# yonahd/krr

Measured on AMD Instinct MI355X. Metric: container-series/sec right-sized (7d@1m) + % of HBM BW, 1/2/4/8 MI355X, higher is better.
Workload: dtype f64; 1 GPU; config2: 10000 containers/rank x 5 pods x 10080 slots (7d@1m), NaN-gapped dense; percentile_mode=linear, cpu_percentile=99, memory_buffer=max x 1.05 (exact decimal, host), containers=10000, slots_per_rank=1008000000, parallelism=shard1 (contiguous container ranges, RCCL gather of 32-B records), records=page-locked host memory, written by the launch

## Files before the change

krr_amd/csrc/krr_geom.h:

```cpp
#pragma once

#include <stdint.h>

#include "krr_plan.h"

namespace krr {

#define KRR_GEOM KRR_HD inline __attribute__((always_inline))

constexpr int kChunkUnits = kUnroll * kWave;

struct SegGeom {
    int64_t a0, a1;
    int64_t s0;
    int64_t i0;
    int64_t nunits;
    int64_t nfull;
    int32_t rem;
    bool head, tail;
    bool part;
    KRR_GEOM bool partial() const { return part; }
    KRR_GEOM int64_t nch() const { return nfull + (partial() ? 1 : 0); }
    KRR_GEOM uint32_t padding() const {
        return partial() ? (uint32_t)(2 * kChunkUnits - 2 * rem - (head ? 1 : 0) - (tail ? 1 : 0)) : 0u;
    }
    KRR_GEOM int64_t slot(int64_t ci, int u, int l) const { return s0 + 2 * (ci * kChunkUnits + u * kWave + l); }
    KRR_GEOM bool edge(int64_t ci, int u, int l) const {
        return partial() && ci == nfull && u == kUnroll - 1 && l == kWave - 1;
    }
};

KRR_GEOM SegGeom seg_geom(int64_t beg, int64_t end) {
    int64_t a0 = (beg + 1) & ~(int64_t)1;
    if (a0 > end) a0 = end;
    int64_t a1 = end & ~(int64_t)1;
    if (a1 < a0) a1 = a0;
    const int64_t i0 = a0 >> 1;
    const int64_t nunits = (a1 >> 1) - i0;
    const int64_t nfull = nunits / kChunkUnits;
    const int64_t rem = nunits - nfull * kChunkUnits;
    const bool head = a0 > beg, tail = a1 < end;
    const bool part = rem > 0 || head || tail;
    return SegGeom{a0, a1, a0 - beg, i0, nunits, nfull, (int32_t)rem, head, tail, part};
}

struct SegCursor {
    uint32_t full;
    int64_t base;
    int lane;
    KRR_GEOM SegCursor(const SegGeom& g, int lane_) : full((uint32_t)g.nfull), base(g.s0), lane(lane_) {}
    KRR_GEOM bool partial() const { return full == 0; }
    KRR_GEOM bool edge_row(int u) const { return partial() && u == kUnroll - 1; }
    KRR_GEOM bool edge(int u) const { return edge_row(u) && lane == kWave - 1; }
    KRR_GEOM int64_t row_base(int u) const { return base + 2 * kWave * u; }
    KRR_GEOM void next() {
        base += 2 * kChunkUnits;
        --full;
    }
};

}
```

krr_amd/csrc/krr_kernels.hip:

```cpp
#include <hip/hip_runtime.h>

#include <stdint.h>
#include <stdio.h>
#include <string.h>

#include <dlfcn.h>
#include <sched.h>
#include <time.h>
#include <unistd.h>
#include <rccl/rccl.h>

#include <new>
#include <type_traits>

#include "krr_amd.h"
#include "krr_device.h"
#include "krr_plan.h"
#include "krr_geom.h"
#include "krr_json.h"

#ifndef KRR_STREAM_DEPTH
#define KRR_STREAM_DEPTH 2
#endif
#ifndef KRR_WSEL_LONG_DEPTH
// ... 1779 lines not shown
    W.fail = 0;
    W.set_window(kKeyNegInf, kKeyPosInf);
#ifdef KRR_DIAG
    for (int d = 0; d < D_WORDS; ++d) W.diag[d] = 0;
    KRR_DIAG_T0(t_begin);
#endif
    int64_t b = beg, e = end;
    asm volatile("" : "+s"(b), "+s"(e));
    const uint32_t pad =
        stream_segment<true, WindowProc<INLINE_FALLBACK>, INLINE_FALLBACK ? KRR_WSEL_LONG_DEPTH : KRR_ONE_SITE_DEPTH>(
            A.vals, b, e, W, lane);
    __syncthreads();
    const uint64_t nnan = W.nan_total() - pad;
    const uint64_t n = A.gaps ? (uint64_t)L - nnan : (uint64_t)L;
    uint32_t flags = 0;
    double result = bitsd(kQuietNaN);
    bool done = false;
#ifdef KRR_DIAG
    KRR_DIAG_T0(t_final);
#endif
    if (W.fail) {
    } else if (n == 0) {
        flags = KRR_FLAG_EMPTY;
        done = true;
    } else if (nnan && !A.gaps) {
        flags = KRR_FLAG_NAN;
        done = true;
    } else {
        const Ranks R = ranks_for(A, n);
        const uint64_t below = W.below_total();
        if (below <= (uint64_t)R.r0 && (uint64_t)R.r1 < below + W.cnt) {
            uint64_t k0, k1;
            if (W.point) {
                k0 = k1 = W.lo;
            } else {
                W.sp.cnt = W.cnt;
                W.sp.bad = 0;
                uint64_t mn = W.lo, mx = W.hi;
                if (W.shrinks == 0) W.sp.buf_minmax(mn, mx);
                const uint32_t Rt = (uint32_t)(W.cnt - ((uint64_t)R.r0 - below));
                if (R.r1 != R.r0) {
                    W.sp.kth_pair(Rt, -1, mn, mx, k0, k1);
                } else {
                    k0 = k1 = W.sp.kth_largest(Rt, mn, mx);
                }
            }
            if (!W.sp.bad) {
                result = finish_value(A, R, k0, k1, beg, end, lane);
                done = true;
            }
        }
    }
#ifdef KRR_DIAG
    {
        const unsigned long long t_end = __builtin_amdgcn_s_memtime();
        W.diag[D_TOTAL] = t_end - t_begin;
        W.diag[D_FINAL] = t_end - t_final;
        W.diag[D_NFALLBACK] = done ? 0ull : 1ull;
        W.diag[D_INSERTED] = W.cnt;
        if (lane == 0 && g_diag)
            for (int d = 0; d < D_WORDS; ++d) g_diag[(size_t)s * D_WORDS + d] = W.diag[d];
    }
#endif
    __syncthreads();
    if (!done) {
        if (lane == 0 && A.stats) atomicAdd(A.stats, 1ull);
        if constexpr (INLINE_FALLBACK) {
            hselect_segment(A, s, smem, lane);
        } else if (lane == 0) {
            A.fail_list[atomicAdd(A.fail_count, 1u)] = s;
        }
        return;
    }
    write_result(A, s, result, n, flags, lane);
    __syncthreads();
}

template <bool LONG>
__device__ __forceinline__ void mid_select_segment(const SelectArgs& A, int64_t s, unsigned char* smem, int lane) {
    if constexpr (KRR_WSEL) wselect_segment<LONG>(A, s, smem, lane);
    else hselect_segment(A, s, smem, lane);
}

__global__ __launch_bounds__(64, KRR_HSEL_WAVES_PER_SIMD) void k_hselect_list(SelectArgs A) {
    extern __shared__ __attribute__((aligned(16))) unsigned char smem[];
    const unsigned int n = __builtin_nontemporal_load(A.fail_count);
    for (unsigned int i = blockIdx.x; i < n; i += gridDim.x) hselect_segment(A, A.fail_list[i], smem, threadIdx.x);
}

enum { SEL_SINGLE = 0, SEL_WINDOW = 1, SEL_WINDOW_LONG = 2 };
constexpr int window_waves(bool longseg) {
    return !KRR_WSEL ? KRR_HSEL_WAVES_PER_SIMD : (longseg ? KRR_HSEL_WAVES_PER_SIMD : KRR_WSEL_WAVES_PER_SIMD);
}
template <int KIND>
__global__ __launch_bounds__(64, KIND == SEL_SINGLE ? KRR_SELECT_WAVES_PER_SIMD : window_waves(KIND == SEL_WINDOW_LONG))
void k_select(SelectArgs A) {
    extern __shared__ __attribute__((aligned(16))) unsigned char smem[];
    if (KIND != SEL_SINGLE && A.fail_reset && blockIdx.x == 0 && threadIdx.x == 0) *A.fail_reset = 0;
    for (int64_t s = blockIdx.x; s < A.S; s += gridDim.x) {
        if constexpr (KIND != SEL_SINGLE) mid_select_segment<KIND == SEL_WINDOW_LONG>(A, xcd_item(s, A.S, A.remap), smem, threadIdx.x);
        else select_segment(A, xcd_item(s, A.S, A.remap), smem, threadIdx.x);
    }
}

struct WindowExportArgs {
    SelectArgs A;
    double ext;
    uint32_t key_cap;
    krr_window_hdr* hdr;
    uint64_t* keys;
};

template <bool LONG>
__device__ __forceinline__ void window_export_segment(const WindowExportArgs& X, int64_t s, unsigned char* smem,
                                                      int lane) {
    const SelectArgs& A = X.A;
    const int64_t beg = A.offs[s], end = A.offs[s + 1];
    const int64_t L = end - beg;
    WindowProc<LONG, true> W;
    W.buf = reinterpret_cast<uint64_t*>(smem + kSelectLdsFixed);
    W.sp.buf = W.buf;
    W.sp.H = reinterpret_cast<uint32_t*>(smem);
    W.sp.small = reinterpret_cast<uint64_t*>(smem + 1024);
    W.sp.lane = lane;
    W.sp.flip = 0;
    W.sp.cnt = 0;
    W.sp.bad = 0;
    W.lane = lane;
    W.cap = A.wcap;
    W.shrinks = 0;
    W.cnt = 0;
    W.below_u = W.nan_u = 0;
    W.below_l = W.nan_l = W.negnan_l = 0;
    W.below_extra = 0;
    W.seen = 0;
    W.L = L;
    W.p_num = A.p_num;
    W.p_den = A.p_den;
    W.fail = 0;
    W.ext_u = X.ext;
    W.set_window(kKeyNegInf, kKeyPosInf);
    int64_t b = (int64_t)uni64((uint64_t)beg), e = (int64_t)uni64((uint64_t)end);
    asm volatile("" : "+s"(b), "+s"(e));
    const uint32_t pad = stream_segment<true, WindowProc<LONG, true>, LONG ? KRR_WSEL_LONG_DEPTH : KRR_ONE_SITE_DEPTH>(
        A.vals, b, e, W, lane);
    __syncthreads();
    const uint64_t nnan = W.fail ? 0 : W.nan_total() - pad;
    const uint64_t n = A.gaps ? (uint64_t)L - nnan : (uint64_t)L;
    const bool has_nan = nnan && !A.gaps;
    if (!W.fail && n > 0 && !has_nan) W.export_shrink(X.key_cap);
    uint32_t flags = 0;
    if (has_nan) W.cnt = 0;
    if (W.fail || (!W.point && W.cnt > X.key_cap)) flags |= KRR_WIN_FAIL;
    if (has_nan) flags |= KRR_FLAG_NAN;
    if (W.point) flags |= KRR_WIN_POINT;
    if (!(flags & (KRR_WIN_FAIL | KRR_WIN_POINT))) {
        uint64_t* row = X.keys + (size_t)s * X.key_cap;
        for (uint32_t i = lane; i < W.cnt; i += kWave) row[i] = W.buf[i];
    }
    const uint64_t below = W.below_total();
    if (lane == 0) {
        krr_window_hdr h;
        h.lo = W.lo;
        h.hi = W.hi;
        h.below = (int64_t)below;
        h.n = (int64_t)n;
        h.cnt = W.cnt;
        h.flags = flags;
        X.hdr[s] = h;
    }
    __syncthreads();
}

template <bool LONG>
__global__ __launch_bounds__(64, window_waves(LONG)) void k_window_export(WindowExportArgs X) {
    extern __shared__ __attribute__((aligned(16))) unsigned char smem[];
    for (int64_t s = blockIdx.x; s < X.A.S; s += gridDim.x) window_export_segment<LONG>(X, xcd_item(s, X.A.S, X.A.remap), smem, threadIdx.x);
}

struct OpAdd64 {
    __device__ uint64_t operator()(uint64_t a, uint64_t b) const { return a + b; }
};
__device__ __forceinline__ uint64_t wave_sum_u64(uint64_t x) {
    return lane_bcast64(wave_scan64(x, 0ull, OpAdd64{}), kWave - 1);
}

struct WindowMergeArgs {
    SelectArgs A;
    int32_t slices;
    int64_t stride;
    const krr_window_hdr* hdr;
    const uint64_t* keys;
    int64_t key_cap;
    unsigned int* miss_count;
};

__global__ __launch_bounds__(64) void k_window_merge(WindowMergeArgs M) {
    extern __shared__ __attribute__((aligned(16))) unsigned char smem[];
    const int lane = threadIdx.x;
    const SelectArgs& A = M.A;
    uint64_t* buf = reinterpret_cast<uint64_t*>(smem + kSelectLdsFixed);
    for (int64_t s = blockIdx.x; s < A.S; s += gridDim.x) {
        const bool has = lane < M.slices;
        krr_window_hdr h;
        if (has) {
            h = M.hdr[(int64_t)lane * M.stride + s];
        } else {
            h.lo = 0;
            h.hi = ~0ull;
            h.below = h.n = 0;
            h.cnt = h.flags = 0;
        }
        const uint64_t n = wave_sum_u64((uint64_t)h.n);
        const uint64_t Lk = wave_max_u64(h.lo), Hk = wave_min_u64(h.hi);
        const bool any_nan = ballot((h.flags & KRR_FLAG_NAN) != 0) != 0;
        const bool any_fail =
            ballot((h.flags & KRR_WIN_FAIL) != 0 || (!(h.flags & KRR_WIN_POINT) && h.cnt > M.key_cap)) != 0;
        uint32_t flags = 0;
        double result = bitsd(kQuietNaN);
        bool miss = false;
        if (any_nan) {
            flags = KRR_FLAG_NAN;
        } else if (n == 0) {
            flags = KRR_FLAG_EMPTY;
        } else if (!rule_covers((int64_t)n, A.ktab, A.ktab_len)) {
            flags = KRR_FLAG_CAPACITY;
        } else if (any_fail || Lk > Hk) {
            miss = true;
        } else {
            const Ranks R = ranks_for(A, n);
            uint64_t cb = wave_sum_u64((uint64_t)h.below);
            uint32_t inr = 0, inr_point = 0;
#pragma unroll 1
            for (int j = 0; j < M.slices; ++j) {
                const uint64_t loj = lane_bcast64(h.lo, j);
                const uint32_t cj = lane_bcast32(h.cnt, j), fj = lane_bcast32(h.flags, j);
                if (fj & KRR_WIN_POINT) {
                    if (loj < Lk) cb += cj;
                    else if (loj <= Hk) inr_point += cj;
                    continue;
                }
                const uint64_t* row = M.keys + ((int64_t)j * M.stride + s) * M.key_cap;
                uint32_t lt = 0;
                for (uint32_t base = 0; base < cj; base += kWave) {
                    const uint32_t i = base + lane;
                    const bool v = i < cj;
                    const uint64_t k = v ? row[i] : 0ull;
                    lt += popc64(ballot(v && k < Lk));
                    const bool in = v && k >= Lk && k <= Hk;
                    const uint64_t m = ballot(in);
                    if (in) buf[inr + lane_prefix(m)] = k;
                    inr += popc64(m);
                }
                cb += lt;
            }
            __syncthreads();
            const uint64_t tot = (uint64_t)inr + inr_point;
            if (cb <= (uint64_t)R.r0 && (uint64_t)R.r1 < cb + tot) {
                uint64_t k0 = Lk, k1 = Lk;
                bool bad = false;
                if (Lk != Hk && inr_point == 0) {
                    SelectProc sp;
                    sp.buf = buf;
                    sp.H = reinterpret_cast<uint32_t*>(smem);
                    sp.small = reinterpret_cast<uint64_t*>(smem + 1024);
                    sp.lane = lane;
                    sp.flip = 0;
                    sp.cnt = inr;
                    sp.bad = 0;
                    uint64_t mn, mx;
                    sp.buf_minmax(mn, mx);
                    const uint32_t Rt = (uint32_t)(inr - ((uint64_t)R.r0 - cb));
                    if (R.r1 != R.r0) sp.kth_pair(Rt, -1, mn, mx, k0, k1);
                    else k0 = k1 = sp.kth_largest(Rt, mn, mx);
                    bad = sp.bad != 0;
                }
                const double a = bitsd(okey_inv(k0));
                if (bad) {
                    miss = true;
                } else if (A.mode == KRR_PCT_SORTED_LOWER) {
                    if (is_zero_bits(dbits(a))) miss = true;
                    else result = a;
                } else {
                    result = np_lerp(a, R.r1 != R.r0 ? bitsd(okey_inv(k1)) : a, R.gamma);
                }
            } else {
                miss = true;
            }
        }
        if (miss) {
            flags = KRR_FLAG_WINDOW_MISS;
            result = bitsd(kQuietNaN);
        }
        if (lane == 0) {
            A.out_v[s] = result;
            A.out_n[s] = (int64_t)n;
            A.out_f[s] = flags;
            if (miss && M.miss_count) atomicAdd(M.miss_count, 1u);
        }
        __syncthreads();
    }
}

struct NanCountProc {
    uint32_t nn;
    __device__ __forceinline__ void chunk(const double2 (&c)[kUnroll]) {
#pragma unroll
        for (int j = 0; j < 2 * kUnroll; ++j) nn += popc64(ballot(__builtin_isnan(slot_val(c, j))));
    }
};

constexpr int kRefBlock = 16;

struct RefArgs {
    const double* vals;
    const int64_t* offs;
    int64_t S;
    int64_t p_num, p_den;
    const int64_t* ktab;
    int64_t ktab_len;
    double* out_v;
    int64_t* out_n;
    uint32_t* out_f;
    int64_t* rec = nullptr;
};

__device__ __forceinline__ double refindex_walk(const double* vals, int64_t beg, int64_t end, uint64_t k, uint64_t n,
                                                int lane) {
    const bool back = k >= n / 2;
    const uint64_t want = back ? n - 1 - k : k;
    const int64_t step = back ? -1 : 1;
    uint64_t run = 0;
    uint64_t found = kQuietNaN;
    bool done = false;
    for (int64_t pos = back ? end - 1 : beg; !done && (back ? pos >= beg : pos < end);
         pos += step * kRefBlock * kWave) {
        uint64_t u[kRefBlock];
#pragma unroll
        for (int b = 0; b < kRefBlock; ++b) {
            const int64_t i = pos + step * (b * kWave + lane);
            u[b] = (i >= beg && i < end) ? dbits(vals[i]) : kQuietNaN;
        }
#pragma unroll
        for (int b = 0; b < kRefBlock; ++b) {
            if (done) break;
            const bool p = !is_nan_bits(u[b]);
            const uint64_t m = ballot(p);
            const uint32_t c = popc64(m);
            if (run + c > want) {
                const uint64_t sel = ballot(p && lane_prefix(m) == (uint32_t)(want - run));
                found = lane_bcast64(u[b], __ffsll((long long)sel) - 1);
                done = true;
            }
            run += c;
        }
    }
    return bitsd(found);
}

template <bool ONE_SITE>
__device__ __forceinline__ void refindex_gaps_segment(const RefArgs& A, int64_t s, int lane) {
    const int64_t beg = A.offs[s], end = A.offs[s + 1];
    NanCountProc C{0};
    C.nn -= stream_segment<ONE_SITE>(A.vals, beg, end, C, lane);
    const uint64_t n = (uint64_t)(end - beg) - C.nn;
    const uint32_t flags = n ? 0u : KRR_FLAG_EMPTY;
    double result = bitsd(kQuietNaN);
    if (n) {
        const uint64_t k = (uint64_t)rule_rank((int64_t)n, A.p_num, A.p_den, A.ktab, A.ktab_len);
        result = refindex_walk(A.vals, beg, end, k, n, lane);
    }
    if (lane == 0) {
        A.out_v[s] = result;
        A.out_n[s] = (int64_t)n;
        A.out_f[s] = flags;
        put_record(A.rec, s, 0, result, n, flags);
    }
}

__global__ __launch_bounds__(64) void k_refindex_gaps(RefArgs A) {
    for (int64_t s = blockIdx.x; s < A.S; s += gridDim.x) refindex_gaps_segment<false>(A, xcd_item(s, A.S, 1), threadIdx.x);
}

__global__ __launch_bounds__(256) void k_refindex_dense(RefArgs A) {
    const int64_t s = (int64_t)blockIdx.x * blockDim.x + threadIdx.x;
    if (s >= A.S) return;
    const int64_t beg = A.offs[s], end = A.offs[s + 1];
    const int64_t n = end - beg;
    if (n <= 0) {
        A.out_v[s] = bitsd(kQuietNaN);
        A.out_n[s] = 0;
        A.out_f[s] = KRR_FLAG_EMPTY;
        return;
    }
    const int64_t k = rule_rank(n, A.p_num, A.p_den, A.ktab, A.ktab_len);
    A.out_v[s] = A.vals[beg + k];
    A.out_n[s] = n;
    A.out_f[s] = 0;
}

struct MaxProc {
    double mx;
    uint32_t nn;
    __device__ __forceinline__ void chunk(const double2 (&c)[kUnroll]) {
#pragma unroll
        for (int j = 0; j < 2 * kUnroll; ++j) {
            const double d = slot_val(c, j);
            mx = fmax(mx, d);
            nn += popc64(ballot(__builtin_isnan(d)));
        }
    }
};

struct OpMaxF64Bits {
    __device__ uint64_t operator()(uint64_t a, uint64_t b) const { return dbits(fmax(bitsd(a), bitsd(b))); }
};
__device__ __forceinline__ double wave_max_f64(double x) {
    return bitsd(lane_bcast64(wave_scan64(dbits(x), kQuietNaN, OpMaxF64Bits{}), kWave - 1));
}

struct MaxArgs {
    const double* vals;
    const int64_t* offs;
    int64_t S;
    int32_t gaps;
    double* out_v;
    int64_t* out_n;
    uint32_t* out_f;
    int64_t* rec = nullptr;
    const double2* fwd_src = nullptr;
    double2* fwd_dst = nullptr;
    int64_t fwd_units = 0;
    int64_t fwd_items = 0;
    int32_t remap = 1;
};

template <class Streamer>
__device__ __forceinline__ void max_segment_with(const MaxArgs& A, int64_t s, int lane, Streamer stream) {
    {
        const int64_t beg = A.offs[s], end = A.offs[s + 1];
        MaxProc M{__builtin_nan(""), 0u};
        M.nn -= stream(M);
        const uint64_t L = (uint64_t)(end - beg);
        const uint64_t n = A.gaps ? L - M.nn : L;
        const double mx = wave_max_f64(M.mx);
        double result = bitsd(kQuietNaN);
        uint32_t flags = 0;
        if (n == 0) {
            flags = KRR_FLAG_EMPTY;
        } else if (M.nn && !A.gaps) {
            flags = KRR_FLAG_NAN;
        } else {
            uint64_t bits = uni64(dbits(mx));
            if (is_zero_bits(bits)) bits = nth_zero_bits(A.vals, beg, end, 0, lane);
            result = bitsd(bits);
        }
        if (lane == 0) {
            A.out_v[s] = result;
            A.out_n[s] = (int64_t)n;
            A.out_f[s] = flags;
            put_record(A.rec, s, 1, result, n, flags);
        }
    }
}

template <bool ONE_SITE>
__device__ __forceinline__ void max_segment(const MaxArgs& A, int64_t s, int lane) {
    const int64_t beg = A.offs[s], end = A.offs[s + 1];
    max_segment_with(A, s, lane, [&](MaxProc& M) { return stream_segment<ONE_SITE>(A.vals, beg, end, M, lane); });
}

__global__ __launch_bounds__(64) void k_max(MaxArgs A) {
    for (int64_t s = blockIdx.x; s < A.S; s += gridDim.x) max_segment<false>(A, xcd_item(s, A.S, A.remap), threadIdx.x);
}

enum { CPU_SELECT = 0, CPU_REF_GAPS = 1, CPU_HSELECT = 2, CPU_HSELECT_LONG = 3 };

constexpr int64_t kFwdItemUnits = 4096;
__device__ __forceinline__ void forward_item(const MaxArgs& M, int64_t i, int lane) {
    const int64_t a = i * kFwdItemUnits;
    const int64_t e = a + kFwdItemUnits < M.fwd_units ? a + kFwdItemUnits : M.fwd_units;
#pragma unroll 1
    for (int64_t u = a + lane; u < e; u += kWave) M.fwd_dst[u] = M.fwd_src[u];
}

template <int CPU_KIND, bool FWD = false>
__global__ __launch_bounds__(64, CPU_KIND == CPU_HSELECT ? window_waves(false)
                                : CPU_KIND == CPU_HSELECT_LONG ? window_waves(true)
                                                               : KRR_SELECT_WAVES_PER_SIMD) void k_simple(SelectArgs A, RefArgs R, MaxArgs M) {
    extern __shared__ __attribute__((aligned(16))) unsigned char smem[];
    const int64_t S_cpu = CPU_KIND == CPU_REF_GAPS ? R.S : A.S;
    const int64_t F = FWD ? M.fwd_items : 0;
    const int64_t total = F + S_cpu + M.S;
    constexpr bool kWindow = CPU_KIND == CPU_HSELECT || CPU_KIND == CPU_HSELECT_LONG;
    if (kWindow && A.fail_reset && blockIdx.x == 0 && threadIdx.x == 0) *A.fail_reset = 0;
    for (int64_t bb = blockIdx.x; bb < total; bb += gridDim.x) {
        if constexpr (FWD) {
            if (bb < F) {
                forward_item(M, bb, threadIdx.x);
                continue;
            }
        }
        const int64_t b = bb - F;
        if (b < S_cpu) {
            const int64_t s = xcd_item(b, S_cpu, A.remap);
            if constexpr (CPU_KIND == CPU_SELECT) select_segment(A, s, smem, threadIdx.x);
            else if constexpr (kWindow) mid_select_segment<CPU_KIND == CPU_HSELECT_LONG>(A, s, smem, threadIdx.x);
            else refindex_gaps_segment<true>(R, s, threadIdx.x);
        } else {
            max_segment<true>(M, xcd_item(b - S_cpu, M.S, M.remap), threadIdx.x);
        }
    }
}

struct MultiArgs {
    const double* vals;
    const int64_t* offs;
    int64_t S;
    int32_t gaps;
    int32_t remap;
    uint32_t cap;
    PctSet ps;
    double* out_v;
    int64_t* out_n;
    uint32_t* out_f;
};

__device__ __forceinline__ SelectArgs pct_args(const MultiArgs& A, int j) {
    return SelectArgs{A.vals, A.offs, A.S, A.ps.mode, A.gaps, A.ps.p_num[j], A.ps.p_den[j], A.ps.q[j], A.ps.ktab[j],
                      A.ps.ktab_len[j]};
}

template <class Streamer>
__device__ __forceinline__ void select_segment_multi_with(const MultiArgs& A, int64_t s, unsigned char* smem,
                                                          int lane, Streamer stream) {
    const int64_t beg = A.offs[s], end = A.offs[s + 1];
    const int64_t L = end - beg;
    const SidePlan sp = plan_side_multi(L, A.ps);
    SelectProc P;
    const Streamed T = select_stream(P, A.vals, beg, L, sp, A.cap, A.gaps, smem, lane, stream, [&](uint64_t n) {
        int64_t rmin = (int64_t)n;
#pragma unroll 1
        for (int j = 0; j < A.ps.n; ++j) {
            const int64_t r = ranks_for(pct_args(A, j), n).r0;
            rmin = r < rmin ? r : rmin;
        }
        return rmin;
    });
    const uint32_t base = T.flags(A.gaps);
    const uint32_t bad_stream = P.bad;
#pragma unroll 1
    for (int j = 0; j < A.ps.n; ++j) {
        P.bad = bad_stream;
        const double result = base ? bitsd(kQuietNaN) : select_value(P, pct_args(A, j), T, beg, end, lane);
        const uint32_t flags = base | (P.bad ? KRR_FLAG_CAPACITY | (P.bad << 8) : 0u);
        if (lane == 0) {
            A.out_v[(int64_t)j * A.S + s] = result;
            A.out_f[(int64_t)j * A.S + s] = flags;
        }
    }
    if (lane == 0) A.out_n[s] = (int64_t)T.n;
    __syncthreads();
}

__device__ __forceinline__ void select_segment_multi(const MultiArgs& A, int64_t s, unsigned char* smem, int lane) {
    const int64_t beg = A.offs[s], end = A.offs[s + 1];
    select_segment_multi_with(A, s, smem, lane, [&](SelectProc& P) {
        int64_t b = beg, e = end;
        asm volatile("" : "+s"(b), "+s"(e));
        return stream_segment<true>(A.vals, b, e, P, lane);
    });
}

__device__ __forceinline__ void refindex_gaps_segment_multi(const MultiArgs& A, int64_t s, int lane) {
    const int64_t beg = A.offs[s], end = A.offs[s + 1];
    NanCountProc C{0};
    C.nn -= stream_segment<true>(A.vals, beg, end, C, lane);
    const uint64_t n = (uint64_t)(end - beg) - C.nn;
#pragma unroll 1
    for (int j = 0; j < A.ps.n; ++j) {
        double result = bitsd(kQuietNaN);
        if (n) {
            const uint64_t k = (uint64_t)rule_rank((int64_t)n, A.ps.p_num[j], A.ps.p_den[j], A.ps.ktab[j],
                                                   A.ps.ktab_len[j]);
            result = refindex_walk(A.vals, beg, end, k, n, lane);
        }
        if (lane == 0) {
            A.out_v[(int64_t)j * A.S + s] = result;
            A.out_f[(int64_t)j * A.S + s] = n ? 0u : KRR_FLAG_EMPTY;
        }
    }
    if (lane == 0) A.out_n[s] = (int64_t)n;
}

__global__ __launch_bounds__(256) void k_refindex_dense_multi(MultiArgs A) {
    const int64_t s = (int64_t)blockIdx.x * blockDim.x + threadIdx.x;
    if (s >= A.S) return;
    const int64_t beg = A.offs[s], end = A.offs[s + 1];
    const int64_t n = end - beg;
    A.out_n[s] = n > 0 ? n : 0;
    for (int j = 0; j < A.ps.n; ++j) {
        double v = bitsd(kQuietNaN);
        if (n > 0) v = A.vals[beg + rule_rank(n, A.ps.p_num[j], A.ps.p_den[j], A.ps.ktab[j], A.ps.ktab_len[j])];
        A.out_v[(int64_t)j * A.S + s] = v;
        A.out_f[(int64_t)j * A.S + s] = n > 0 ? 0u : KRR_FLAG_EMPTY;
    }
}

template <int CPU_KIND>
__global__ __launch_bounds__(64, KRR_SELECT_WAVES_PER_SIMD) void k_simple_multi(MultiArgs A, MaxArgs M) {
    static_assert(CPU_KIND == CPU_SELECT || CPU_KIND == CPU_REF_GAPS, "the window kernels follow one rank");
    extern __shared__ __attribute__((aligned(16))) unsigned char smem[];
    const int64_t total = A.S + M.S;
    for (int64_t b = blockIdx.x; b < total; b += gridDim.x) {
        if (b < A.S) {
            const int64_t s = xcd_item(b, A.S, A.remap);
            if constexpr (CPU_KIND == CPU_SELECT) select_segment_multi(A, s, smem, threadIdx.x);
            else refindex_gaps_segment_multi(A, s, threadIdx.x);
        } else {
            max_segment<true>(M, xcd_item(b - A.S, M.S, M.remap), threadIdx.x);
        }
    }
}

__global__ __launch_bounds__(256) void k_pack_records(int64_t S, const double* __restrict__ cv,
                                                      const int64_t* __restrict__ cn,
                                                      const uint32_t* __restrict__ cf,
                                                      const double* __restrict__ mv,
                                                      const int64_t* __restrict__ mn,
                                                      const uint32_t* __restrict__ mf,
                                                      int64_t* __restrict__ rec) {
    const int64_t s = (int64_t)blockIdx.x * blockDim.x + threadIdx.x;
    if (s >= S) return;
    longlong2 a, b;
    a.x = (long long)dbits(cv[s]);
    a.y = (long long)dbits(mv[s]);
    b.x = (long long)((uint64_t)cn[s] | ((uint64_t)cf[s] << 48));
    b.y = (long long)((uint64_t)mn[s] | ((uint64_t)mf[s] << 48));
    reinterpret_cast<longlong2*>(rec)[2 * s] = a;
    reinterpret_cast<longlong2*>(rec)[2 * s + 1] = b;
}

struct OpOr32 {
    __device__ uint32_t operator()(uint32_t a, uint32_t b) const { return a | b; }
};

struct GroupMaxArgs {
    int64_t G;
    const int64_t* goffs;
    int32_t rows;
    int64_t N;
    const double* in_v;
    const int64_t* in_n;
    const uint32_t* in_f;
    double* out_v;
    int64_t* out_n;
    uint32_t* out_f;
    int64_t* out_arg;
    int64_t* rec;
};

__global__ __launch_bounds__(64) void k_group_max(GroupMaxArgs A) {
    const int lane = threadIdx.x;
    constexpr int64_t kNone = 0x7FFFFFFFFFFFFFFFll;
    for (int64_t g = blockIdx.x; g < A.G; g += gridDim.x) {
        const int64_t a0 = A.goffs[g];
        int64_t a = a0, e = A.goffs[g + 1];
        a = a < 0 ? 0 : a;
        e = e > A.N ? A.N : e;
#pragma unroll 1
        for (int r = 0; r < A.rows; ++r) {
            const double* v = A.in_v + (int64_t)r * A.N;
            const uint32_t* f = A.in_f + (int64_t)r * A.N;
            uint64_t best = 0;
            int64_t best_i = kNone, bad_i = kNone;
            uint64_t cnt = 0;
            uint32_t fo = 0, have = 0;
            for (int64_t i = a + lane; i < e; i += kWave) {
                const uint32_t fl = f[i];
                if (fl & KRR_FLAG_EMPTY) continue;
                have = 1;
                fo |= fl;
                cnt += (uint64_t)A.in_n[i];
                const uint64_t u = dbits(v[i]);
                if ((fl & (KRR_FLAG_NAN | KRR_FLAG_CAPACITY)) || is_nan_bits(u)) {
                    if (bad_i == kNone) bad_i = i;
                } else {
                    const uint64_t key = okey(is_zero_bits(u) ? 0ull : u);
                    if (key > best) {
                        best = key;
                        best_i = i;
                    }
                }
            }
            const bool any = ballot(have != 0) != 0;
            const uint64_t kmax = wave_max_u64(best);
            const int64_t win = (int64_t)wave_min_u64(best == kmax ? (uint64_t)best_i : (uint64_t)kNone);
            const int64_t bad = (int64_t)wave_min_u64((uint64_t)bad_i);
            const uint64_t n = lane_bcast64(wave_scan64(cnt, 0ull, OpAdd64{}), kWave - 1);
            const uint32_t flags = lane_bcast32(wave_scan32(fo, 0u, OpOr32{}), kWave - 1);
            if (lane == 0) {
                double result = bitsd(kQuietNaN);
                uint32_t of = KRR_FLAG_EMPTY;
                int64_t arg = -1;
                if (any) {
                    of = flags;
                    if (bad != kNone) {
                        arg = bad - a0;
                    } else if (win != kNone) {
                        result = v[win];
                        arg = win - a0;
                    }
                }
                const int64_t o = (int64_t)r * A.G + g;
                A.out_v[o] = result;
                A.out_f[o] = of;
                if (A.out_arg) A.out_arg[o] = arg;
                if (r == 0) A.out_n[g] = (int64_t)n;
                put_record(A.rec, g, 0, result, n, of);
            }
        }
    }
}

__global__ void k_maxlen(const int64_t* __restrict__ offs, int64_t S, unsigned long long* out) {
    uint64_t m = 0;
    for (int64_t s = (int64_t)blockIdx.x * blockDim.x + threadIdx.x; s < S;
         s += (int64_t)gridDim.x * blockDim.x) {
        const int64_t L = offs[s + 1] - offs[s];
        m = (uint64_t)L > m ? (uint64_t)L : m;
    }
    m = wave_max_u64(m);
    if ((threadIdx.x & 63) == 0) atomicMax(out, (unsigned long long)m);
}

struct SketchGeom {
    uint32_t m, nbins, width, base;
    uint64_t low_bits;
    int32_t e_lo;
};

__host__ __device__ inline SketchGeom sketch_geom(const krr_sketch_params& p) {
    SketchGeom g;
    g.m = (uint32_t)p.mantissa_bits;
    g.nbins = (uint32_t)p.octaves << g.m;
    g.width = g.nbins + 4;
    g.e_lo = p.min_exponent;
    g.base = (uint32_t)(p.min_exponent + 1023) << g.m;
    g.low_bits = (uint64_t)(p.min_exponent + 1023) << 52;
    return g;
}

__device__ __forceinline__ uint32_t sketch_bin(const SketchGeom& g, uint64_t x) {
    const uint64_t mag = x & ~kSignBit;
    const uint32_t u = (uint32_t)(mag >> (52 - g.m)) - g.base;
    uint32_t bin = u < g.nbins ? 3u + u : (mag < g.low_bits ? 2u : 3u + g.nbins);
    bin = (x & kSignBit) ? 0u : bin;
    bin = mag == 0 ? 1u : bin;
    return bin;
}

struct SketchProc {
    uint32_t* h;
    SketchGeom g;
    uint32_t nan_l;
    double vmin, vmax;
    __device__ __forceinline__ void chunk(const double2 (&c)[kUnroll]) {
#pragma unroll
        for (int j = 0; j < 2 * kUnroll; ++j) {
            const double d = slot_val(c, j);
            const uint64_t x = dbits(d);
            const bool nan = __builtin_isnan(d);
            nan_l += nan ? 1u : 0u;
            vmin = fmin(vmin, d);
            vmax = fmax(vmax, d);
            const uint32_t bin = sketch_bin(g, x);
            if (!nan) atomicAdd(&h[bin], 1u);
            asm volatile("" ::: "memory");
        }
    }
};

struct OpMinF64Bits {
    __device__ uint64_t operator()(uint64_t a, uint64_t b) const { return dbits(fmin(bitsd(a), bitsd(b))); }
};

struct SketchBuildArgs {
    const double* vals;
    const int64_t* offs;
    int64_t S;
    int32_t gaps;
    SketchGeom g;
    uint32_t* counts;
    double* vmin;
    double* vmax;
    uint32_t* flags;
};

__global__ __launch_bounds__(64) void k_sketch_build(SketchBuildArgs A) {
    extern __shared__ __attribute__((aligned(16))) unsigned char smem[];
    uint32_t* h = reinterpret_cast<uint32_t*>(smem);
    const int lane = threadIdx.x;
    for (int64_t s = blockIdx.x; s < A.S; s += gridDim.x) {
        const int64_t beg = A.offs[s], end = A.offs[s + 1];
        for (uint32_t i = lane; i < A.g.width; i += kWave) h[i] = 0;
        __syncthreads();
        SketchProc P;
        P.h = h;
        P.g = A.g;
        P.nan_l = 0;
        P.vmin = bitsd(kQuietNaN);
        P.vmax = bitsd(kQuietNaN);
        const uint32_t pad = stream_segment<true>(A.vals, beg, end, P, lane);
        __syncthreads();
        const uint64_t nnan = wave_sum_u32(P.nan_l) - pad;
        const double mn = bitsd(lane_bcast64(wave_scan64(dbits(P.vmin), kQuietNaN, OpMinF64Bits{}), kWave - 1));
        const double mx = bitsd(lane_bcast64(wave_scan64(dbits(P.vmax), kQuietNaN, OpMaxF64Bits{}), kWave - 1));
        uint4* dst = reinterpret_cast<uint4*>(A.counts + (size_t)s * A.g.width);
        const uint4* src = reinterpret_cast<const uint4*>(h);
        for (uint32_t i = lane; i < A.g.width / 4; i += kWave) dst[i] = src[i];
        if (lane == 0) {
            A.vmin[s] = mn;
            A.vmax[s] = mx;
            A.flags[s] = (nnan && !A.gaps) ? KRR_FLAG_NAN : 0u;
        }
        __syncthreads();
    }
}

struct SketchQueryArgs {
    int64_t S;
    SketchGeom g;
    const uint32_t* counts;
    const double* vmin;
    const double* vmax;
    int32_t mode;
    int64_t p_num, p_den;
    double q;
    double* out_v;
    int64_t* out_n;
    uint32_t* out_f;
    const int64_t* ktab = nullptr;
    int64_t ktab_len = 0;
};

__device__ __forceinline__ double sketch_value(const SketchGeom& g, uint32_t b, uint64_t r, uint64_t before, uint32_t c,
                                               double mn, double mx, uint64_t n, uint32_t& flags) {
    if (r == 0) return mn;
    if (r == n - 1) return mx;
    const double f = ((double)(r - before) + 0.5) / (double)c;
    double lo, hi;
    if (b == 1) return 0.0;
    if (b == 0) {
        lo = mn;
        hi = 0.0;
        flags |= KRR_FLAG_SKETCH_RANGE;
    } else if (b == 2) {
        lo = 0.0;
        hi = ldexp(1.0, g.e_lo);
        flags |= KRR_FLAG_SKETCH_RANGE;
    } else if (b == 3 + g.nbins) {
        lo = ldexp(1.0, g.e_lo + (int)(g.nbins >> g.m));
        hi = mx;
        flags |= KRR_FLAG_SKETCH_RANGE;
    } else {
        const uint32_t i = b - 3;
        const int E = g.e_lo + (int)(i >> g.m);
        const double j = (double)(i & ((1u << g.m) - 1u));
        const double step = ldexp(1.0, E - (int)g.m);
        lo = ldexp(1.0, E) + j * step;
        hi = lo + step;
    }
    double v = lo + f * (hi - lo);
    v = v < mn ? mn : v;
    v = v > mx ? mx : v;
    return v;
}

__global__ __launch_bounds__(64) void k_sketch_query(SketchQueryArgs A) {
    const int lane = threadIdx.x;
    for (int64_t s = blockIdx.x; s < A.S; s += gridDim.x) {
        const uint32_t* h = A.counts + (size_t)s * A.g.width;
        const uint32_t W = A.g.width;
        const uint32_t per = (W + kWave - 1) / kWave;
        const uint32_t b0 = (uint32_t)lane * per;
        uint32_t t = 0;
        for (uint32_t j = 0; j < per; ++j) t += b0 + j < W ? h[b0 + j] : 0u;
        const uint32_t incl = wave_scan32(t, 0u, OpAdd32{});
// ... 3418 lines not shown
```

Baseline: 8.416 million container-series/s.

## Locate reference-index rank via per-group non-NaN prefix counts instead of full walk

During the NaN-counting pass, each chunk's non-NaN count is accumulated into per-lane group prefix sums, splitting the full chunks into at most one group per wave lane. The rank lookup then uses a ballot over these prefixes to find the group holding the k-th valid value and walks only that group, or the trailing remainder. This replaces the previous walk from the nearer end of the segment, which could scan up to half of it. It adds bookkeeping to every chunk of the counting pass and relies on the head slot and chunk alignment matching the stream geometry.

New measurement: 8.293 million container-series/s. 1.5% lower.

```diff
diff --git a/krr_amd/csrc/krr_geom.h b/krr_amd/csrc/krr_geom.h
--- a/krr_amd/csrc/krr_geom.h
+++ b/krr_amd/csrc/krr_geom.h
@@ -59,4 +59,41 @@
     }
 };
 
+constexpr int64_t kChunkSlots = 2 * kChunkUnits;
+
+KRR_GEOM int64_t ref_group_chunks(int64_t nfull) {
+    const int64_t G = (nfull + kWave - 1) / kWave;
+    return G < 1 ? 1 : G;
 }
+KRR_GEOM int64_t ref_ngroups(int64_t nfull) {
+    const int64_t G = ref_group_chunks(nfull);
+    return (nfull + G - 1) / G;
+}
+struct SlotRange {
+    int64_t lo, hi;
+};
+KRR_GEOM SlotRange ref_group_range(const SegGeom& g, int64_t G, int64_t j) {
+    const int64_t c1 = (j + 1) * G < g.nfull ? (j + 1) * G : g.nfull;
+    return SlotRange{g.a0 + j * G * kChunkSlots, g.a0 + c1 * kChunkSlots};
+}
+KRR_GEOM SlotRange ref_rest_range(const SegGeom& g, int64_t end) {
+    return SlotRange{g.a0 + g.nfull * kChunkSlots, end};
+}
+struct RefGroupCursor {
+    uint32_t full;
+    uint32_t G;
+    uint32_t left;
+    uint32_t group;
+    KRR_GEOM explicit RefGroupCursor(int64_t nfull)
+        : full((uint32_t)nfull), G((uint32_t)ref_group_chunks(nfull)), left(G), group(0) {}
+    KRR_GEOM bool in_full() const { return full != 0; }
+    KRR_GEOM void next() {
+        --full;
+        if (--left == 0 || full == 0) {
+            ++group;
+            left = G;
+        }
+    }
+};
+
+}
diff --git a/krr_amd/csrc/krr_kernels.hip b/krr_amd/csrc/krr_kernels.hip
--- a/krr_amd/csrc/krr_kernels.hip
+++ b/krr_amd/csrc/krr_kernels.hip
@@ -2105,15 +2105,31 @@
     }
 }
 
-struct NanCountProc {
-    uint32_t nn;
+struct RefCountProc {
+    uint32_t nn = 0;
+    uint32_t run = 0;
+    uint32_t cum = 0;
+    uint64_t head = kQuietNaN;
+    RefGroupCursor at;
+    int lane;
+    __device__ __forceinline__ RefCountProc(const SegGeom& g, int lane_) : at(g.nfull), lane(lane_) {}
     __device__ __forceinline__ void chunk(const double2 (&c)[kUnroll]) {
-#pragma unroll
-        for (int j = 0; j < 2 * kUnroll; ++j) nn += popc64(ballot(__builtin_isnan(slot_val(c, j))));
+        uint32_t t = 0;
+#pragma unroll
+        for (int j = 0; j < 2 * kUnroll; ++j) t += popc64(ballot(__builtin_isnan(slot_val(c, j))));
+        nn += t;
+        if (at.in_full()) {
+            run += (uint32_t)kChunkSlots - t;
+            if ((uint32_t)lane == at.group) cum = run;
+            at.next();
+        } else {
+            head = lane_bcast64(dbits(c[kUnroll - 1].x), kWave - 1);
+        }
     }
 };
 
 constexpr int kRefBlock = 16;
+static_assert(kRefBlock * kWave == kChunkSlots, "one chunk is one locate step");
 
 struct RefArgs {
     const double* vals;
@@ -2128,21 +2144,16 @@
     int64_t* rec = nullptr;
 };
 
-__device__ __forceinline__ double refindex_walk(const double* vals, int64_t beg, int64_t end, uint64_t k, uint64_t n,
-                                                int lane) {
-    const bool back = k >= n / 2;
-    const uint64_t want = back ? n - 1 - k : k;
-    const int64_t step = back ? -1 : 1;
+__device__ __forceinline__ double refindex_walk(const double* vals, int64_t lo, int64_t hi, uint64_t want, int lane) {
     uint64_t run = 0;
     uint64_t found = kQuietNaN;
     bool done = false;
-    for (int64_t pos = back ? end - 1 : beg; !done && (back ? pos >= beg : pos < end);
-         pos += step * kRefBlock * kWave) {
+    for (int64_t pos = lo; !done && pos < hi; pos += kRefBlock * kWave) {
         uint64_t u[kRefBlock];
 #pragma unroll
         for (int b = 0; b < kRefBlock; ++b) {
-            const int64_t i = pos + step * (b * kWave + lane);
-            u[b] = (i >= beg && i < end) ? dbits(vals[i]) : kQuietNaN;
+            const int64_t i = pos + b * kWave + lane;
+            u[b] = i < hi ? dbits(vals[i]) : kQuietNaN;
         }
 #pragma unroll
         for (int b = 0; b < kRefBlock; ++b) {
@@ -2161,17 +2172,34 @@
     return bitsd(found);
 }
 
+__device__ __forceinline__ double refindex_locate(const double* vals, const SegGeom& g, int64_t end,
+                                                  const RefCountProc& C, uint64_t k, int lane) {
+    const bool h = !is_nan_bits(C.head);
+    if (h && k == 0) return bitsd(C.head);
+    const uint64_t kk = k - (h ? 1u : 0u);
+    const uint64_t hit = ballot((uint32_t)lane < C.at.group && (uint64_t)C.cum > kk);
+    uint32_t before = C.run;
+    SlotRange r = ref_rest_range(g, end);
+    if (hit) {
+        const int j = __ffsll((long long)hit) - 1;
+        before = j ? lane_bcast32(C.cum, j - 1) : 0u;
+        r = ref_group_range(g, C.at.G, j);
+    }
+    return refindex_walk(vals, r.lo, r.hi, kk - before, lane);
+}
+
 template <bool ONE_SITE>
 __device__ __forceinline__ void refindex_gaps_segment(const RefArgs& A, int64_t s, int lane) {
     const int64_t beg = A.offs[s], end = A.offs[s + 1];
-    NanCountProc C{0};
+    const SegGeom g = seg_geom(beg, end);
+    RefCountProc C(g, lane);
     C.nn -= stream_segment<ONE_SITE>(A.vals, beg, end, C, lane);
     const uint64_t n = (uint64_t)(end - beg) - C.nn;
     const uint32_t flags = n ? 0u : KRR_FLAG_EMPTY;
     double result = bitsd(kQuietNaN);
     if (n) {
         const uint64_t k = (uint64_t)rule_rank((int64_t)n, A.p_num, A.p_den, A.ktab, A.ktab_len);
-        result = refindex_walk(A.vals, beg, end, k, n, lane);
+        result = refindex_locate(A.vals, g, end, C, k, lane);
     }
     if (lane == 0) {
         A.out_v[s] = result;
@@ -2377,7 +2405,8 @@
 
 __device__ __forceinline__ void refindex_gaps_segment_multi(const MultiArgs& A, int64_t s, int lane) {
     const int64_t beg = A.offs[s], end = A.offs[s + 1];
-    NanCountProc C{0};
+    const SegGeom g = seg_geom(beg, end);
+    RefCountProc C(g, lane);
     C.nn -= stream_segment<true>(A.vals, beg, end, C, lane);
     const uint64_t n = (uint64_t)(end - beg) - C.nn;
 #pragma unroll 1
@@ -2386,7 +2415,7 @@
         if (n) {
             const uint64_t k = (uint64_t)rule_rank((int64_t)n, A.ps.p_num[j], A.ps.p_den[j], A.ps.ktab[j],
                                                    A.ps.ktab_len[j]);
-            result = refindex_walk(A.vals, beg, end, k, n, lane);
+            result = refindex_locate(A.vals, g, end, C, k, lane);
         }
         if (lane == 0) {
             A.out_v[(int64_t)j * A.S + s] = result;
```
